# qwerty35/lsc_dr_planner

Hardware: AMD Instinct MI355X
Metric: qp_solves_per_sec (higher is better)
Workload: dtype f64; 1 GPU; configs[1]: 64 agents x M=5 x ~20 LSC half-spaces/seg, fp64 -- 64 agents/GPU x M=5 segments x 20 LSC neighbours (dim=3, forest swarm after 3 warm-up replans), fp64: dual active-set phase (one workgroup per QP) with the batched PDIP behind it for what it leaves; batch_seed=1000, precision=f64, row_format=f64, collective_backend=none (single process), agents_per_gpu=64, agents_total=64, ranks=1, distinct_devices=1, launch=single process, segments=5, lsc_neighbours=20, dim=3, rows_per_qp=1074, allgather=False, pipeline=False, hip_graph=False

## Files before the change

### lsc_dr_planner_amd/csrc/lscqp_das.hpp

```cpp
#pragma once
#include <hip/hip_runtime.h>
#include <stdint.h>

#include "lscqp_kernel.hpp"
#include "lscqp_launch.hpp"

#pragma clang fp contract(on)

namespace lscqp_das {

using lscqp::DevClass;
using lscqp::KQ;

constexpr double kTolP = 1e-9;
constexpr double kTolD = 1e-9;
constexpr int kMaxK = 32;

__host__ __device__ constexpr size_t table_stride(int M) { return (size_t)(3 + 6 * M) * (size_t)(6 * M); }
__host__ __device__ constexpr int num_pairs(int M, int dim) { return dim * (6 * M + 5 * M + 4 * M + M * (M - 1) / 2); }

struct Layout {
    int P, NX, kmax, NPAIR;
    int o_hdr, o_sfc, o_c, o_cu, o_lam, o_plo, o_phi, o_pix, o_W, o_L, o_u, o_r, o_arhs, o_acoef, o_aint, o_red, o_ctl, o_wb, o_dq, o_C, o_rows, o_tl, n_stage, total;
    __host__ __device__ static constexpr Layout make(int M, int dim, int kmax, int cacheC, int stage_rows = 0) {
        Layout s{};
        s.P = 6 * M, s.NX = dim * s.P, s.kmax = kmax, s.NPAIR = num_pairs(M, dim);
        int o = 0;
        auto take = [&](int n) { const int at = o; o += (n + 1) & ~1; return at; };
        s.o_hdr = take(32);
        s.o_sfc = take(6 * M);
        s.o_c = take(3 * s.P), s.o_cu = take(s.NX), s.o_lam = take(s.NX);
        s.o_plo = take(s.NPAIR), s.o_phi = take(s.NPAIR), s.o_pix = take((s.NPAIR + 1) / 2);
        s.o_W = take((kmax + 1) * s.NX);
        s.o_L = take(kmax * (kmax + 1));
        s.o_u = take(kmax + 1), s.o_r = take(kmax + 4), s.o_arhs = take(kmax + 1);
        s.o_acoef = take(3 * (kmax + 1));
        s.o_aint = take(2 * (kmax + 1) + 2);
        s.o_red = take(2 * 24);
        s.o_ctl = take(8);
        s.o_wb = take(8);
        s.o_dq = take(36);
        s.o_C = take(cacheC ? s.P * s.P : 0);
        s.n_stage = stage_rows;
        s.o_rows = take(4 * stage_rows);
#ifdef LSCQP_DAS_TIMING
        s.o_tl = take(16);
#endif
        s.total = o;
        return s;
    }
};

__device__ __forceinline__ double wave_max(double v) { return lscqp::wave_max(v); }
__device__ __forceinline__ double wave_min(double v) { return -lscqp::wave_max(-v); }
__device__ __forceinline__ double wave_sum(double v) { return lscqp::wave_sum(v); }
template <int CTRL, int ROW_MASK>
__device__ __forceinline__ int dpp_min_i32(int v) {
    return min(v, __builtin_amdgcn_update_dpp(2147483647, v, CTRL, ROW_MASK, 0xf, false));
}
__device__ __forceinline__ int wave_min_i32(int v) {
    v = dpp_min_i32<0x111, 0xf>(v);
    v = dpp_min_i32<0x112, 0xf>(v);
    v = dpp_min_i32<0x114, 0xf>(v);
    v = dpp_min_i32<0x118, 0xf>(v);
    v = dpp_min_i32<0x142, 0xa>(v);
    v = dpp_min_i32<0x143, 0xc>(v);
    return __builtin_amdgcn_readlane(v, 63);
}
__device__ __forceinline__ void wave_argmin(double& v, int& id) {
    const double vm = wave_min(v);
    id = wave_min_i32((v == vm) ? id : 2147483647);
    v = vm;
}
__device__ __forceinline__ int fdiv(int a, float inv_b) { return (int)(((float)a + 0.5f) * inv_b); }

#ifndef LSCQP_DAS_FULL_SYNC
#define LSCQP_DAS_WAVE_SYNC()                                   \
    do {                                                        \
        __builtin_amdgcn_fence(__ATOMIC_RELEASE, "wavefront");  \
        __builtin_amdgcn_wave_barrier();                        \
        __builtin_amdgcn_fence(__ATOMIC_ACQUIRE, "wavefront");  \
    } while (0)
#define LSCQP_DAS_BARRIER()                                                           \
    do {                                                                              \
        if constexpr (NW > 1) asm volatile("s_waitcnt lgkmcnt(0)\n\ts_barrier" ::: "memory"); \
        else asm volatile("s_waitcnt lgkmcnt(0)" ::: "memory");                       \
    } while (0)
#else
#define LSCQP_DAS_WAVE_SYNC()                                           \
    do {                                                                \
        __builtin_amdgcn_fence(__ATOMIC_SEQ_CST, "workgroup");          \
        asm volatile("s_waitcnt vmcnt(0) lgkmcnt(0)" ::: "memory");     \
        __builtin_amdgcn_wave_barrier();                                \
        __builtin_amdgcn_fence(__ATOMIC_SEQ_CST, "workgroup");          \
    } while (0)
#define LSCQP_DAS_BARRIER()                                             \
    do {                                                                \
        __builtin_amdgcn_fence(__ATOMIC_SEQ_CST, "workgroup");          \
        asm volatile("s_waitcnt vmcnt(0) lgkmcnt(0)" ::: "memory");     \
        if constexpr (NW > 1) __syncthreads();                          \
        __builtin_amdgcn_fence(__ATOMIC_SEQ_CST, "workgroup");          \
    } while (0)
#endif

#ifdef LSCQP_DAS_TIMING
#ifndef LSCQP_DAS_CYCLES
#define LSCQP_DAS_CYCLES das_cycles
#endif
__device__ unsigned long long LSCQP_DAS_CYCLES[16];
#define DAS_T_DECL()                                                                                                                  \
    unsigned long long* const das_tl_ = reinterpret_cast<unsigned long long*>(smem + L.o_tl);                                         \
    if (threadIdx.x == 0)                                                                                                             \
        for (int i_ = 0; i_ < 16; i_++) das_tl_[i_] = 0;                                                                              \
    unsigned long long tprev_ = __builtin_readcyclecounter()
#define DAS_T(slot)                                                        \
    do {                                                                   \
        if ((LSCQP_DAS_TIMING >> (slot)) & 1) {                            \
            const unsigned long long now_ = __builtin_readcyclecounter();  \
            if (tid == 0) das_tl_[slot] += now_ - tprev_;                  \
            tprev_ = now_;                                                 \
        }                                                                  \
    } while (0)
#ifndef LSCQP_DAS_TIMING_MIN_STEPS
#define LSCQP_DAS_TIMING_MIN_STEPS 0
#endif
#define DAS_T_FLUSH()                                                                    \
    do {                                                                                 \
        if (tid == 0 && steps >= LSCQP_DAS_TIMING_MIN_STEPS)                             \
            for (int i_ = 0; i_ < 16; i_++) atomicAdd(&LSCQP_DAS_CYCLES[i_], das_tl_[i_]);   \
    } while (0)
#else
#define DAS_T_DECL() \
    do {             \
    } while (0)
#define DAS_T(slot) \
    do {            \
    } while (0)
#define DAS_T_FLUSH() \
    do {              \
    } while (0)
#endif

#define LSCQP_DAS_GLOBAL __attribute__((address_space(1)))
#define LSCQP_DAS_KERNARGS()                                                                                                            \
    double ka_wb0 = cls.world_min[0], ka_wb1 = cls.world_min[1], ka_wb2 = cls.world_min[2];                                            \
    double ka_wb3 = cls.world_max[0], ka_wb4 = cls.world_max[1], ka_wb5 = cls.world_max[2];                                            \
    double ka_dt = cls.dt, ka_q2s = cls.q2s, ka_w_t = cls.w_t, ka_w_c = cls.w_c, ka_comm_range = cls.comm_range;                               \
    int ka_use_sfc = cls.use_sfc, ka_rsfc = cls.rsfc;                                                                                  \
    const int32_t* const ka_order = cls.order;                                                                                        \
    LSCQP_DAS_GLOBAL const uint64_t* ka_roffs = (LSCQP_DAS_GLOBAL const uint64_t*)row_offsets;                                         \
    LSCQP_DAS_GLOBAL const double* ka_sfc = (LSCQP_DAS_GLOBAL const double*)sfc;                                                       \
    asm volatile(""                                                                                                                    \
                 : "+s"(ka_wb0), "+s"(ka_wb1), "+s"(ka_wb2), "+s"(ka_wb3), "+s"(ka_wb4), "+s"(ka_wb5), "+s"(ka_dt), "+s"(ka_q2s),      \
                   "+s"(ka_w_t), "+s"(ka_w_c), "+s"(ka_comm_range), "+s"(ka_use_sfc), "+s"(ka_rsfc), "+s"(ka_roffs), "+s"(ka_sfc)                   \
                 : "s"(ka_order), "s"(tab), "s"(hdr), "s"(rows), "s"(n), "s"(cap), "s"(kmax), "s"(max_steps),        \
                   "s"(cacheC), "s"(stage_rows), "s"(x_init), "s"(x_out), "s"(obj_out), "s"(status_out), "s"(info_out))

struct Row {
    int ent[3];
    double coef[3];
    double rhs;
};
__device__ __forceinline__ int ent_axis(int e) { return e >> 16; }
__device__ __forceinline__ int ent_cp(int e) { return e & 0xffff; }

__device__ __forceinline__ double ccol(const int* ea, const double* ca, int kx, int cp, const double* __restrict__ Cm, int P) {
    double s = 0.0;
#pragma unroll
    for (int i = 0; i < 3; i++) {
        const double v = Cm[(size_t)ent_cp(ea[i]) * P + cp];
        s += ((ent_axis(ea[i]) == kx) ? ca[i] : 0.0) * v;
    }
    return s;
}
__device__ __forceinline__ double cdot(const int* ea, const double* ca, const int* eb, const double* cb, const double* __restrict__ Cm, int P) {
    double s = 0.0;
#pragma unroll
    for (int i = 0; i < 3; i++) {
#pragma unroll
        for (int j = 0; j < 3; j++) {
            const double v = Cm[(size_t)ent_cp(ea[i]) * P + ent_cp(eb[j])];
            s += ((ent_axis(ea[i]) == ent_axis(eb[j])) ? ca[i] * cb[j] : 0.0) * v;
        }
    }
    return s;
}

#ifndef LSCQP_DAS_KU1
#define LSCQP_DAS_KU1 2
#endif
#ifndef LSCQP_DAS_WPE1
#define LSCQP_DAS_WPE1 3
#endif
#ifndef LSCQP_DAS_WPES
#define LSCQP_DAS_WPES 4
#endif
enum DasVerdict { kDasSolved = 0, kDasInfeasible = 1, kDasHandedOver = 2 };

template <int NW, bool F32, bool SCREEN = false, bool PEEL = false>
__global__ __launch_bounds__(64 * NW, (SCREEN ? LSCQP_DAS_WPES : NW == 1 ? LSCQP_DAS_WPE1 : 1)) void das_kernel(DevClass cls, int M, int dim, int es, int cap, int kmax, int max_steps, int cacheC, int stage_rows, int behind,
                                                      const double* __restrict__ tab, int64_t n, const lscqp_header* __restrict__ hdr,
                                                      const lscqp_row* __restrict__ rows, const uint64_t* __restrict__ row_offsets,
                                                      const lscqp_box* __restrict__ sfc, const double* __restrict__ x_init, double* __restrict__ x_out,
                                                      double* __restrict__ obj_out, int32_t* __restrict__ status_out, lscqp_info* __restrict__ info_out) {
    extern __shared__ __attribute__((aligned(16))) double smem[];
    constexpr int T = 64 * NW;
    constexpr int kU = SCREEN ? 4 : (NW == 1) ? LSCQP_DAS_KU1 : 4;
    constexpr int kMaxNL = 0x7fffffff;
    const int64_t k0 = blockIdx.x;
    if (k0 >= n) return;
    const int64_t q = cls.order ? (int64_t)cls.order[k0] : k0;
#define LSCQP_DAS_PROLOGUE 0
#define LSCQP_DAS_STEP_PATH 0
#define LSCQP_DAS_END(verdict_) return
#include "lscqp_das_body.inc"
#undef LSCQP_DAS_END
#undef LSCQP_DAS_STEP_PATH
#undef LSCQP_DAS_PROLOGUE
}

}
```

### lsc_dr_planner_amd/csrc/lscqp_das_body.inc

```
#if LSCQP_DAS_PROLOGUE
#define DAS_CLS(f) ka_##f
#else
#define DAS_CLS(f) cls.f
#endif
    const int tid = threadIdx.x, lane = tid & 63, wv = tid >> 6;
#ifdef LSCQP_DAS_LAYOUT
    constexpr Layout L = LSCQP_DAS_LAYOUT;
#else
    const Layout L = Layout::make(M, dim, kmax, cacheC, stage_rows);
#endif
    DAS_T_DECL();
    const int P = L.P, NX = L.NX, NPAIR = L.NPAIR;
    const int kcap = L.kmax;
    double* const H_ = smem + L.o_hdr;
    double* const sfc_ = smem + L.o_sfc;
    double* const c_ = smem + L.o_c;
    double* const cu_ = smem + L.o_cu;
    double* const lam_ = smem + L.o_lam;
    double* const plo_ = smem + L.o_plo;
    double* const phi_ = smem + L.o_phi;
    int* const pix_ = reinterpret_cast<int*>(smem + L.o_pix);
    double* const W_ = smem + L.o_W;
    double* const Jm_ = smem + L.o_L;
    double* const u_ = smem + L.o_u;
// ... 138 lines not shown
    }
    const double dt = DAS_CLS(dt);
    const double org0 = Hd->p0[0], org1 = Hd->p0[1], org2 = Hd->p0[2];
    const double* const org = Hd->p0;
    int ts = Hd->terminal_segments;
    if (ts <= 0) {
        const double g0 = Hd->goal[0] - org0, g1 = Hd->goal[1] - org1, g2 = Hd->goal[2] - org2;
        ts = (int)((M * dt - sqrt(g0 * g0 + g1 * g1 + g2 * g2) / Hd->nominal_velocity + 1e-9) / dt);
        if (ts < 1) ts = 1;
    }
    if (ts > M) ts = M;
    const double q2s = DAS_CLS(q2s), wt2 = 2.0 * DAS_CLS(w_t);
    const double* const tb = tab + (size_t)(ts - 1) * table_stride(M);
    const double* const U1 = tb, * const U2 = tb + P, * const G1 = tb + 2 * P, * const Cg = tb + 3 * P;
    const bool comm_on = DAS_CLS(comm_range) > 0;
    const double rho_pair = 0.5 * DAS_CLS(comm_range) - Hd->radius;
    const double rho_wp = 0.5 * DAS_CLS(comm_range) - 1e-5;
#if !LSCQP_DAS_PROLOGUE
    const int nL = n_obs * P;
#endif
    const float iP = 1.0f / (float)P;
    const bool staged = stage_rows > 0 && nL <= stage_rows;
    bool rows_in_lds = false;

#if LSCQP_DAS_PROLOGUE
    constexpr int NE = 4;
    double tu1[NE], tu2[NE], tg1[NE];
#pragma unroll
    for (int i = 0; i < NE; i++) {
        const int e = tid + i * T < NX ? tid + i * T : 0;
        const int cp = e - P * fdiv(e, iP);
        tu1[i] = U1[cp], tu2[i] = U2[cp], tg1[i] = G1[cp];
    }
#else
    auto fetch_row = [&](int j, double& x, double& y, double& z, double& w) {
        if constexpr (F32) {
            const float4 f = reinterpret_cast<const float4*>(rows)[roff + (uint64_t)j];
            x = f.x, y = f.y, z = f.z, w = f.w;
        } else {
            const double4 d = *reinterpret_cast<const double4*>(&rows[roff + (uint64_t)j]);
            x = d.x, y = d.y, z = d.z, w = d.w;
        }
    };
    constexpr int NE = 4;
    double tu1[NE], tu2[NE], tg1[NE];
#pragma unroll
    for (int i = 0; i < NE; i++) {
        const int e = tid + i * T;
        if (e < NX) {
            const int cp = e - P * fdiv(e, iP);
            tu1[i] = U1[cp], tu2[i] = U2[cp], tg1[i] = G1[cp];
        }
    }
    double px[kU], py[kU], pz[kU], pw[kU];
#pragma unroll
    for (int u = 0; u < kU; u++) px[u] = py[u] = pz[u] = 0.0, pw[u] = -1.0;
    if (nL > 0) {
#pragma unroll
        for (int u = 0; u < kU; u++) {
            const int j = tid + u * T;
            fetch_row(j < nL ? j : 0, px[u], py[u], pz[u], pw[u]);
        }
    }
#endif

    constexpr int kCPre = (NW == 4 && !PEEL && !SCREEN) ? 6 : 0;
    double cpre[kCPre > 0 ? kCPre : 1];
#if LSCQP_DAS_PROLOGUE
    const bool c_fits = kCPre > 0 && P * P <= kCPre * T;
    const bool c_prefetched = c_fits && cacheC;
#else
    const bool c_prefetched = kCPre > 0 && cacheC && P * P <= kCPre * T;
    const bool c_fits = c_prefetched;
#endif
    if constexpr (kCPre > 0) {
        if (c_fits) {
#pragma unroll
            for (int i = 0; i < kCPre; i++) {
                const int e = tid + i * T;
                cpre[i] = Cg[e < P * P ? e : 0];
            }
        }
    }
#if LSCQP_DAS_STEP_PATH & 2
#ifndef LSCQP_DAS_LAYOUT
#error "LSCQP_DAS_STEP_PATH & 2 needs the compile-time carve"
#endif
    static_assert(NW > 1, "the first pass's barrier publishes the table");
    constexpr bool kTableEarly = kCPre > 0 && L.P * L.P <= kCPre * T;
    static_assert(!kTableEarly || LSCQP_DAS_PROLOGUE, "the table is stored from cpre[]: it needs the prologue that always loads it");
#else
    constexpr bool kTableEarly = false;
#endif

    bool empty = false;
    const double hv_c = dt * 0.2, ha_c = dt * dt * 0.05;
    for (int r0 = tid; r0 < NPAIR; r0 += kPB * T) {
        if (r0 != tid) {
#pragma unroll
            for (int u = 0; u < kPB; u++) pwr[u] = pairs_g[min(r0 + u * T, NPAIR - 1)];
        }
#pragma unroll
        for (int u = 0; u < kPB; u++) {
            if ((r0 - tid) + u * T >= NPAIR) break;
            const int r = r0 + u * T;
            const int w0 = pwr[u].x, w1 = pwr[u].y;
            const int fam = w1 & 3, k = (w1 >> 2) & 3, m = (w1 >> 4) & 15;
            const bool last = (w1 >> 8) & 1, rs = (w1 >> 9) & 1;
            const double ok_ = org[k], wlo = wb_[k], whi = wb_[3 + k], wpk = Hd->next_waypoint[k] - ok_;
            const double hv = Hd->vmax[k] * hv_c, ha = Hd->amax[k] * ha_c;
            double lo = wlo - ok_, hi = whi - ok_;
            if (DAS_CLS(rsfc) && rs) {
                lo = -100.0 - ok_;
                hi = 100.0 - ok_;
            }
            if (DAS_CLS(use_sfc)) {
                lo = fmax(lo, sfcl[m].bmin[k] - ok_);
                hi = fmin(hi, sfcl[m].bmax[k] - ok_);
            }
            const double clo = fmax(lo, fmax(-rho_pair, wpk - rho_wp)), chi = fmin(hi, fmin(rho_pair, wpk + rho_wp));
            lo = (comm_on && last) ? clo : lo;
            hi = (comm_on && last) ? chi : hi;
            const double hs = fam == 1 ? hv : fam == 2 ? ha : rho_pair;
            lo = fam == 0 ? lo : -hs;
            hi = fam == 0 ? hi : hs;
            if (r < NPAIR) {
                if (fam == 0 && (w0 >> 24) != 0 && lo > hi) empty = true;
                plo_[r] = lo, phi_[r] = hi;
                pix_[r] = w0;
            }
        }
    }
#pragma unroll
    for (int i = 0; i < NE; i++) {
        const int e = tid + i * T;
        if (e < NX) {
            const int k = fdiv(e, iP), cp = e - k * P;
            const double c1 = Hd->v0[k] * dt * 0.2;
            const double c2 = Hd->a0[k] * dt * dt * 0.05 + 2.0 * c1;
            const double fixv = (cp == 1) ? c1 : (cp == 2) ? c2 : 0.0;
            const double cv = fixv - c1 * tu1[i] - c2 * tu2[i] + wt2 * (Hd->goal[k] - org[k]) * tg1[i];
            c_[e] = cv;
            cu_[e] = cv;
        }
    }
    if (dim == 2)
        for (int e = tid; e < P; e += T) c_[2 * P + e] = 0.0;
#if LSCQP_DAS_STEP_PATH & 2
    {
        double2* const J2 = reinterpret_cast<double2*>(Jm_);
        for (int e = tid; e < kcap * LDL / 2; e += T) J2[e] = make_double2(0.0, 0.0);
    }
#endif
#if LSCQP_DAS_PROLOGUE
    const bool empty_w = __ballot(empty) != 0;
    if constexpr (NW > 1) {
        if (lane == 0) red_[20 + wv] = empty_w ? 1.0 : 0.0;
    }
    LSCQP_DAS_BARRIER();
    bool empty_g = empty_w;
    if constexpr (NW > 1) {
        empty_g = false;
#pragma unroll
        for (int w = 0; w < NW; w++) empty_g = empty_g || red_[20 + w] != 0.0;
    }
#else
    if (tid == 0) ctl_[4] = 0.0;
    LSCQP_DAS_BARRIER();
    if (empty) ctl_[4] = 1.0;
    LSCQP_DAS_BARRIER();
#endif
#if LSCQP_DAS_PROLOGUE
    if (empty_g)
#else
    if (ctl_[4] != 0.0)
#endif
    {
        double ov = 0.0;
        if (wv == 0) {
            for (int r = lane; r < NPAIR; r += 64)
                if ((pix_[r] >> 24) != 0) ov = fmax(ov, plo_[r] - phi_[r]);
            ov = wave_max(ov);
        }
        infeasible_out(0, ov);
        LSCQP_DAS_END(kDasInfeasible);
    }
    DAS_T(1);

    auto translate = [&](int j, double x, double y, double z, double w, double& nx, double& ny, double& nz, double& b) -> bool {
        nx = x, ny = y, nz = (dim == 3) ? z : 0.0;
        b = (dim == 3) ? w - (x * org0 + y * org1 + z * org2) : w - (x * org0 + y * org1 + 0.0);
        return !(x * x + y * y + z * z < 1e-10) && (j - P * fdiv(j, iP)) >= 3;
    };
    auto load_row = [&](int j, double& nx, double& ny, double& nz, double& b) -> bool {
        if (rows_in_lds) {
            nx = Sx_[j], ny = Sy_[j], nz = Sz_[j], b = Sb_[j];
            return b != -1.0 || nx != 0.0 || ny != 0.0 || nz != 0.0;
        }
        double x, y, z, w;
        fetch_row(j, x, y, z, w);
        return translate(j, x, y, z, w, nx, ny, nz, b);
    };
    auto pair_val = [&](int pk, const double* vec) -> double {
        const int type = pk >> 24, e0 = (pk >> 12) & 0xfff, e1 = pk & 0xfff;
        const int i0 = (type == 4) ? e1 : e0 + max(type - 1, 0);
        const int i1 = (type == 3) ? e0 + 1 : e0;
        const double a1 = (type <= 1) ? 0.0 : (type == 3) ? -2.0 : -1.0;
        const double a2 = (type == 3) ? 1.0 : 0.0;
        const double v0 = vec[i0], v1 = vec[i1], v2 = vec[e0];
        return (v0 + a1 * v1) + a2 * v2;
    };
    auto ent_of = [&](int e) -> int {
        const int k = fdiv(e, iP);
        return (k << 16) | (e - k * P);
    };
    auto decode = [&](int rid, Row& R) {
        R.ent[0] = R.ent[1] = R.ent[2] = 0;
        R.coef[0] = R.coef[1] = R.coef[2] = 0.0;
        if (rid < nL) {
            const int cp = rid - P * fdiv(rid, iP);
            double nx, ny, nz, b;
            (void)load_row(rid, nx, ny, nz, b);
            R.ent[0] = cp, R.ent[1] = (1 << 16) | cp, R.ent[2] = (2 << 16) | cp;
            R.coef[0] = nx, R.coef[1] = ny, R.coef[2] = (dim == 3) ? nz : 0.0;
            R.rhs = b;
            return;
        }
        const int s = rid - nL, r = s >> 1, pk = pix_[r];
        const int type = pk >> 24, e0 = (pk >> 12) & 0xfff, e1 = pk & 0xfff;
        const double sg = (s & 1) ? -1.0 : 1.0;
        R.rhs = (s & 1) ? -phi_[r] : plo_[r];
        const bool t1 = type == 1, t2 = type == 2, t3 = type == 3;
        R.ent[0] = ent_of(t1 ? e0 : t2 ? e0 + 1 : t3 ? e0 + 2 : e1);
        R.ent[1] = t1 ? 0 : ent_of(t3 ? e0 + 1 : e0);
        R.ent[2] = t3 ? ent_of(e0) : 0;
        R.coef[0] = sg;
        R.coef[1] = t1 ? 0.0 : t3 ? -2.0 * sg : -sg;
        R.coef[2] = t3 ? sg : 0.0;
    };
    auto row_dot = [&](const int* ent, const double* coef, const double* vec) -> double {
        return coef[0] * vec[ent_axis(ent[0]) * P + ent_cp(ent[0])] + coef[1] * vec[ent_axis(ent[1]) * P + ent_cp(ent[1])] +
               coef[2] * vec[ent_axis(ent[2]) * P + ent_cp(ent[2])];
    };

    bool first_pass = true;
    auto pass_local = [&](double& bv, int& bi) {
        bv = 1e300;
        bi = 0x7fffffff;
        auto see = [&](double slack, int id) {
            slack = (slack == slack) ? slack : -1e308;
            const bool lt = slack < bv;
            bv = lt ? slack : bv;
            bi = lt ? id : bi;
        };
        auto eval = [&](int j0, const double* rx, const double* ry, const double* rz, const double* rb) {
#pragma unroll
            for (int u = 0; u < kU; u++) {
                const int j = j0 + u * T, jc = j < nL ? j : 0;
                const int cp = jc - P * fdiv(jc, iP);
                see(rx[u] * c_[cp] + ry[u] * c_[P + cp] + rz[u] * c_[2 * P + cp] - rb[u], j);
            }
        };
        auto prep = [&](int j0, const double* x, const double* y, const double* z, const double* w, double* rx, double* ry, double* rz, double* rb) {
#pragma unroll
            for (int u = 0; u < kU; u++) {
                const int j = j0 + u * T, jc = j < nL ? j : 0;
                const bool ok = translate(jc, x[u], y[u], z[u], w[u], rx[u], ry[u], rz[u], rb[u]) && j < nL;
                rx[u] = ok ? rx[u] : 0.0, ry[u] = ok ? ry[u] : 0.0, rz[u] = ok ? rz[u] : 0.0, rb[u] = ok ? rb[u] : -1.0;
            }
        };
        auto stage = [&](int j0, const double* rx, const double* ry, const double* rz, const double* rb) {
#pragma unroll
            for (int u = 0; u < kU; u++) {
                const int j = j0 + u * T;
                if (j < nL) Sx_[j] = rx[u], Sy_[j] = ry[u], Sz_[j] = rz[u], Sb_[j] = rb[u];
            }
        };
        double rx[kU], ry[kU], rz[kU], rb[kU];
        if (first_pass) {
            prep(tid, px, py, pz, pw, rx, ry, rz, rb);
            if (staged) stage(tid, rx, ry, rz, rb);
            eval(tid, rx, ry, rz, rb);
            for (int j0 = tid + kU * T; kMaxNL > kU * T && j0 < nL; j0 += kU * T) {
                double x[kU], y[kU], z[kU], w[kU];
#pragma unroll
                for (int u = 0; u < kU; u++) fetch_row(j0 + u * T < nL ? j0 + u * T : 0, x[u], y[u], z[u], w[u]);
                prep(j0, x, y, z, w, rx, ry, rz, rb);
                if (staged) stage(j0, rx, ry, rz, rb);
                eval(j0, rx, ry, rz, rb);
            }
        } else if (rows_in_lds) {
#if LSCQP_DAS_STEP_PATH & 1
            for (int j0 = tid; j0 < nL; j0 += kU * T) {
                double lx[kU], ly[kU], lz[kU], lb[kU];
#pragma unroll
                for (int u = 0; u < kU; u++) {
                    const int j = j0 + u * T, jc = j < nL ? j : 0;
                    lx[u] = Sx_[jc], ly[u] = Sy_[jc], lz[u] = Sz_[jc], lb[u] = Sb_[jc];
                }
#pragma unroll
                for (int u = 0; u < kU; u++) {
                    const bool in = j0 + u * T < nL;
                    rx[u] = in ? lx[u] : 0.0, ry[u] = in ? ly[u] : 0.0, rz[u] = in ? lz[u] : 0.0, rb[u] = in ? lb[u] : -1.0;
                }
                eval(j0, rx, ry, rz, rb);
            }
#else
            for (int j0 = tid; j0 < nL; j0 += kU * T) {
#pragma unroll
                for (int u = 0; u < kU; u++) {
                    const int j = j0 + u * T, jc = j < nL ? j : 0;
                    rx[u] = Sx_[jc], ry[u] = Sy_[jc], rz[u] = Sz_[jc], rb[u] = (j < nL) ? Sb_[jc] : 1e300;
                    if (!(j < nL)) rx[u] = ry[u] = rz[u] = 0.0, rb[u] = -1.0;
                }
                eval(j0, rx, ry, rz, rb);
            }
#endif
        } else {
            for (int j0 = tid; j0 < nL; j0 += kU * T) {
                double x[kU], y[kU], z[kU], w[kU];
#pragma unroll
                for (int u = 0; u < kU; u++) fetch_row(j0 + u * T < nL ? j0 + u * T : 0, x[u], y[u], z[u], w[u]);
                prep(j0, x, y, z, w, rx, ry, rz, rb);
                eval(j0, rx, ry, rz, rb);
            }
        }
        first_pass = false;
        DAS_T(8);
        for (int r0 = tid; r0 < NPAIR; r0 += 2 * T) {
            const int r1 = r0 + T, r1c = r1 < NPAIR ? r1 : r0;
            const int pk0 = pix_[r0], pk1 = pix_[r1c];
            const double lo0 = plo_[r0], hi0 = phi_[r0], lo1 = plo_[r1c], hi1 = phi_[r1c];
            const double d0 = pair_val(pk0, c_), d1 = pair_val(pk1, c_);
            const bool on0 = (pk0 >> 24) != 0, on1 = (pk1 >> 24) != 0 && r1 < NPAIR;
            see(on0 ? d0 - lo0 : 1.0, nL + 2 * r0);
            see(on0 ? hi0 - d0 : 1.0, nL + 2 * r0 + 1);
            see(on1 ? d1 - lo1 : 1.0, nL + 2 * r1);
            see(on1 ? hi1 - d1 : 1.0, nL + 2 * r1 + 1);
        }
        DAS_T(9);
    };
    auto pass_combine = [&](const double* rb_, double& bv, int& bi) {
        bv = rb_[0], bi = reinterpret_cast<const int*>(rb_ + 4)[0];
#pragma unroll
        for (int w = 1; w < NW; w++) {
            const double ov = rb_[w];
            const int oi = reinterpret_cast<const int*>(rb_ + 4)[w];
            if (ov < bv || (ov == bv && oi < bi)) bv = ov, bi = oi;
        }
    };
    auto pass = [&](double& best, int& bid) {
        const bool was_first = first_pass;
        double bv;
        int bi;
        pass_local(bv, bi);
#if LSCQP_DAS_STEP_PATH & 2
        if constexpr (kTableEarly) {
            if (was_first) {
#pragma unroll
                for (int i = 0; i < kCPre; i++) {
                    const int e = tid + i * T;
                    if (e < P * P) Cc_[e] = cpre[i];
                }
            }
        }
#endif
        wave_argmin(bv, bi);
        if constexpr (NW > 1) {
            double* const rb_ = red_ + 24 * par;
            par ^= 1;
            if (lane == 0) {
                rb_[wv] = bv;
                reinterpret_cast<int*>(rb_ + 4)[wv] = bi;
            }
            LSCQP_DAS_BARRIER();
            pass_combine(rb_, bv, bi);
        } else if (staged && was_first) {
            LSCQP_DAS_BARRIER();
        }
        if (staged) rows_in_lds = true;
        best = bv, bid = bi;
    };

    const double* Cm = kTableEarly ? Cc_ : Cg;
    auto factor_remove = [&](int k_, int l_) -> bool {
        bool ok = true;
        if (wv == 0) {
            const int k = __builtin_amdgcn_readfirstlane(k_), l = __builtin_amdgcn_readfirstlane(l_);
            const bool mine = lane < k;
            const int c = mine ? lane : 0;
            const int cn = c - (c > l ? 1 : 0);
            double carry = Jm_[l * LDL + c];
            double a = Jm_[l * LDL + l];
            for (int j = l; j < k - 1; j++) {
                const double x = Jm_[(j + 1) * LDL + c];
                const double b = Jm_[(j + 1) * LDL + l];
                const double r2 = a * a + b * b;
                if (!(r2 > 1e-280)) ok = false;
                const double ir = rsqrt(fmax(r2, 1e-300));
                const double ca = a * ir, sb = b * ir;
                const double fin = ca * x - sb * carry;
                carry = ca * carry + sb * x;
                a = r2 * ir;
                if (mine && lane != l) Jm_[j * LDL + cn] = fin;
            }
            if (mine) Jm_[(k - 1) * LDL + lane] = 0.0, Jm_[lane * LDL + k - 1] = 0.0;
            LSCQP_DAS_WAVE_SYNC();
        }
        return ok;
    };
    auto solve_factor = [&](int k_, double vi, double* yy) -> double {
        const int k = __builtin_amdgcn_readfirstlane(k_);
        const bool mine = lane < k;
        const int ll = min(lane, kcap - 1);
        vi = mine ? vi : 0.0;
        double yi = 0.0, ri = 0.0;
        for (int j0 = 0; j0 < k; j0 += 8) {
            double Jr[8];
#pragma unroll
            for (int t_ = 0; t_ < 8; t_++) Jr[t_] = Jm_[ll * LDL + min(j0 + t_, kcap)];
#pragma unroll
            for (int t_ = 0; t_ < 8; t_++) yi += Jr[t_] * lscqp::bcast(vi, j0 + t_);
        }
        yi = mine ? yi : 0.0;
        if (yy) *yy = wave_sum(yi * yi);
        for (int j0 = 0; j0 < k; j0 += 8) {
            double Jc[8];
#pragma unroll
            for (int t_ = 0; t_ < 8; t_++) Jc[t_] = Jm_[min(j0 + t_, kcap - 1) * LDL + ll];
#pragma unroll
            for (int t_ = 0; t_ < 8; t_++) ri += Jc[t_] * lscqp::bcast(yi, j0 + t_);
        }
        ri = mine ? ri : 0.0;
        if (lane < kcap + 4) r_[lane] = ri;
        return ri;
    };
    auto add_columns = [&](int k, const double* wts, const double* base) {
        for (int e = tid; e < NX; e += T) {
            double a = base ? base[e] : c_[e];
            for (int j = 0; j < k; j++) a += wts[j] * W_[(size_t)j * NX + e];
            c_[e] = a;
        }
    };

    const int NZA = 3 * (M - 1) + (es ? 1 : 3);
    auto finish_local = [&](int k, double& rd, double& gs, double& part) {
#if LSCQP_DAS_PROLOGUE
        const double dt = wb_[6], q2s = wb_[7], ka_w_t = ctl_[4], ka_w_c = red_[44], wt2 = 2.0 * ka_w_t;
#endif
        if (k > 0) {
            for (int e = tid; e < NX; e += T) lam_[e] = 0.0;
            LSCQP_DAS_BARRIER();
            if (tid == 0) {
                for (int j = 0; j < k; j++)
#pragma unroll
                    for (int t_ = 0; t_ < 3; t_++) {
                        const int en = aint_[4 * j + 1 + t_];
                        lam_[ent_axis(en) * P + ent_cp(en)] += u_[j] * acoef_[3 * j + t_];
                    }
            }
            LSCQP_DAS_BARRIER();
        }
        rd = 0.0, gs = 0.0;
        for (int zi = tid; zi < dim * NZA; zi += T) {
            const int kx = zi / NZA, a = zi - kx * NZA;
            const bool last = es && a == 3 * (M - 1);
            const int m = last ? M - 1 : a / 3, j = last ? 0 : a % 3;
            const double c1 = Hd->v0[kx] * dt * 0.2;
            const double c2 = Hd->a0[kx] * dt * dt * 0.05 + 2.0 * c1;
            const double gk = Hd->goal[kx] - org[kx];
            auto seg = [&](int mm, double* g, double* g0, double* lm) {
                const double* cc = &c_[kx * P + 6 * mm];
                const double v0 = cc[0], v1 = cc[1], v2 = cc[2], v3 = cc[3], v4 = cc[4], v5 = cc[5];
                lscqp::static_for<0, 6>([&](auto Ic) {
                    constexpr int i = decltype(Ic)::value;
                    g[i] = q2s * (KQ(i, 0) * v0 + KQ(i, 1) * v1 + KQ(i, 2) * v2 + KQ(i, 3) * v3 + KQ(i, 4) * v4 + KQ(i, 5) * v5);
                    g0[i] = (mm == 0) ? q2s * (KQ(i, 1) * c1 + KQ(i, 2) * c2) : 0.0;
                    lm[i] = (k > 0) ? lam_[kx * P + 6 * mm + i] : 0.0;
                });
                if (mm >= M - ts) {
                    g[5] += wt2 * (v5 - gk);
                    g0[5] += -wt2 * gk;
                }
            };
            double g[6], g0[6], lm[6];
            seg(m, g, g0, lm);
            double cf, cg, c0;
            if (last) {
                cf = (g[3] - lm[3]) + (g[4] - lm[4]) + (g[5] - lm[5]), cg = g[3] + g[4] + g[5], c0 = g0[3] + g0[4] + g0[5];
            } else {
                const double gs_ = j == 0 ? g[3] : j == 1 ? g[4] : g[5], ls_ = j == 0 ? lm[3] : j == 1 ? lm[4] : lm[5], g0s = j == 0 ? g0[3] : j == 1 ? g0[4] : g0[5];
                cf = gs_ - ls_, cg = gs_, c0 = g0s;
            }
            if (m + 1 < M) {
                seg(m + 1, g, g0, lm);
                const double w0 = (j == 2) ? 1.0 : 0.0, w1 = (j == 1) ? -1.0 : (j == 2) ? 2.0 : 0.0, w2 = (j == 0) ? 1.0 : (j == 1) ? -4.0 : 4.0;
                cf += w0 * (g[0] - lm[0]) + w1 * (g[1] - lm[1]) + w2 * (g[2] - lm[2]);
                cg += w0 * g[0] + w1 * g[1] + w2 * g[2];
                c0 += w0 * g0[0] + w1 * g0[1] + w2 * g0[2];
            }
            rd = fmax(rd, fabs(cf));
            gs = fmax(gs, fmax(fabs(cg), fabs(c0)));
        }
        part = 0.0;
        for (int lv = tid - (NW > 1 ? 64 : 0); lv < dim * M; lv += T) {
            if (lv < 0) continue;
            const int kx = lv / M, m = lv - kx * M;
            const double* cc = &c_[kx * P + 6 * m];
            const double j0 = (cc[3] - cc[0]) - 3.0 * (cc[2] - cc[1]);
            const double j1 = (cc[4] - cc[1]) - 3.0 * (cc[3] - cc[2]);
            const double j2 = (cc[5] - cc[2]) - 3.0 * (cc[4] - cc[3]);
            const double quad = 0.2 * (j0 * j0 + j2 * j2) + (2.0 / 15.0) * j1 * j1 + 0.2 * (j0 * j1 + j1 * j2) + (1.0 / 15.0) * j0 * j2;
            double pp = 0.5 * q2s * 3600.0 * quad;
            const double ok_ = org[kx];
            double corr = 0;
            const double s0 = cc[0] + ok_, s1 = cc[1] + ok_, s2 = cc[2] + ok_, s3 = cc[3] + ok_, s4 = cc[4] + ok_, s5 = cc[5] + ok_;
#pragma unroll 1
            for (int i = 0; i < 6; i++) {
                const double* dr = dq_ + 6 * i;
                double r = 0;
                r += dr[0] * s0, r += dr[1] * s1, r += dr[2] * s2, r += dr[3] * s3, r += dr[4] * s4, r += dr[5] * s5;
                corr += r * (cc[i] + ok_);
            }
            pp += DAS_CLS(w_c) * corr;
            const double dgoal = cc[5] - (Hd->goal[kx] - ok_);
            pp += (m >= M - ts) ? DAS_CLS(w_t) * dgoal * dgoal : 0.0;
            part += pp;
        }
    };
    auto finish_combine = [&](const double* rb_, double& rd, double& gs, double& part) {
        rd = rb_[8], gs = rb_[12], part = rb_[16];
#pragma unroll
        for (int w = 1; w < NW; w++) rd = fmax(rd, rb_[8 + w]), gs = fmax(gs, rb_[12 + w]), part += rb_[16 + w];
    };
    auto finish_verdict = [&](double rd, double gs, double part, double& res_d, double& obj) {
        res_d = (part == part && fabs(part) < 1e300) ? rd / fmax(1.0, gs) : 1e300;
        obj = part;
    };
    auto finish = [&](int k, double& res_d, double& obj) {
        double rd, gs, part;
        finish_local(k, rd, gs, part);
        lscqp::wave_reduce3<lscqp::OpMax, lscqp::OpMax, lscqp::OpSum>(rd, gs, part);
        if constexpr (NW > 1) {
            double* const rb_ = red_ + 24 * par;
            par ^= 1;
            if (lane == 0) rb_[8 + wv] = rd, rb_[12 + wv] = gs, rb_[16 + wv] = part;
            LSCQP_DAS_BARRIER();
            finish_combine(rb_, rd, gs, part);
        }
        finish_verdict(rd, gs, part, res_d, obj);
    };

    int k = 0, steps = 0, why = LSCQP_DAS_WHY_VERIFICATION;
    bool polished = false, solved = false, haveC = false, haveJ = false, proven = false;
    double res_p = 0.0, res_d = 0.0, obj = 0.0;
    auto write_out = [&]() {
        for (int e = tid; e < NX; e += T) x_out[q * NX + e] = c_[e] + org[fdiv(e, iP)];
        if (tid == 0) {
            obj_out[q] = obj;
            status_out[q] = LSCQP_STATUS_OPTIMAL;
            if (info_out) {
                info_out[q].iterations = steps;
                info_out[q].flags = LSCQP_INFO_ACTIVE_SET;
                info_out[q].res_primal = res_p;
                info_out[q].res_dual = res_d;
                info_out[q].gap = 0.0;
            }
        }
    };
    double best;
    int bid;
    bool peeled = false;
    if constexpr (PEEL || SCREEN) {
        pass(best, bid);
        DAS_T(2);
        if (!(best < -kTolP)) {
            res_p = fmax(0.0, -best);
            finish(0, res_d, obj);
            DAS_T(4);
            if (res_d <= kTolD) write_out();
            else hand_over(0, LSCQP_DAS_WHY_VERIFICATION);
            DAS_T(7);
            DAS_T_FLUSH();
            LSCQP_DAS_END(res_d <= kTolD ? kDasSolved : kDasHandedOver);
        }
        peeled = true;
    }
    for (;;) {
        if (!((PEEL || SCREEN) && peeled)) {
            pass(best, bid);
            DAS_T(steps == 0 ? 2 : 3);
        }
        peeled = false;
        if (!(best < -kTolP)) {
            res_p = fmax(0.0, -best);
            finish(k, res_d, obj);
            DAS_T(4);
            if (res_d <= kTolD) {
                solved = true;
                break;
            }
            if (polished || k == 0) break;
            LSCQP_DAS_BARRIER();
            add_columns(k, u_, cu_);
            LSCQP_DAS_BARRIER();
            if (wv == 0) {
                const double rho = (lane < k) ? arhs_[lane] - row_dot(&aint_[4 * lane + 1], &acoef_[3 * lane], c_) : 0.0;
                const double du = solve_factor(k, rho, nullptr);
                const double un = (lane < k) ? u_[lane] + du : 0.0;
                const double umax = wave_max(fabs(un));
                const double neg = wave_max((lane < k && un < -1e-12 * umax) ? 1.0 : 0.0);
                if (lane < k) u_[lane] = fmax(un, 0.0);
                if (lane == 0) ctl_[7] = neg;
            }
            LSCQP_DAS_BARRIER();
            if (ctl_[7] != 0.0) {
                why = LSCQP_DAS_WHY_MULTIPLIER;
                break;
            }
            add_columns(k, r_, nullptr);
            LSCQP_DAS_BARRIER();
            polished = true;
            continue;
        }
        polished = false;
        if constexpr (SCREEN) break;
        if (k >= kmax) {
            why = LSCQP_DAS_WHY_ROWS;
            break;
        }
#if LSCQP_DAS_STEP_PATH & 2
        (void)haveJ, (void)haveC;
#else
        if (!haveJ) {
            if (wv == 0)
                for (int e = lane; e < kcap * LDL; e += 64) Jm_[e] = 0.0;
            haveJ = true;
        }
#endif
        if (!kTableEarly && cacheC && !haveC) {
            bool copied = false;
            if constexpr (kCPre > 0) {
                if (c_prefetched) {
#pragma unroll
                    for (int i = 0; i < kCPre; i++) {
                        const int e = tid + i * T;
                        if (e < P * P) Cc_[e] = cpre[i];
                    }
                    copied = true;
                }
            }
            if (!copied)
                for (int e = tid; e < P * P; e += T) Cc_[e] = Cg[e];
            haveC = true;
            Cm = Cc_;
            LSCQP_DAS_BARRIER();
        }
        Row Rp;
        decode(bid, Rp);
        if (tid == 0) {
            aint_[4 * kcap] = bid;
            for (int t = 0; t < 3; t++) aint_[4 * kcap + 1 + t] = Rp.ent[t], acoef_[3 * kcap + t] = Rp.coef[t];
            arhs_[kcap] = Rp.rhs;
            ctl_[3] = 0.0;
        }
        auto compute_wp = [&](int first_thread, int n_threads) {
            for (int e = tid - first_thread; e < NX; e += n_threads) {
                if (e < 0) continue;
                const int kx = fdiv(e, iP), cp = e - kx * P;
                W_[(size_t)k * NX + e] = ccol(Rp.ent, Rp.coef, kx, cp, Cm, P);
            }
        };
        if constexpr (NW == 1) compute_wp(0, T);
        DAS_T(5);
        double spp = 0.0;
        bool stop = false, first_step = true;
        for (;;) {
            steps++;
            if (steps > max_steps) {
                stop = true;
                why = LSCQP_DAS_WHY_STEPS;
                break;
            }
            if (NW > 1 && first_step && wv != 0) compute_wp(64, T - 64);
            if (wv == 0 && __builtin_amdgcn_readfirstlane(k) == 0) {
                if (first_step) spp = cdot(Rp.ent, Rp.coef, Rp.ent, Rp.coef, Cm, P);
                const double sp = row_dot(Rp.ent, Rp.coef, c_) - Rp.rhs;
                const double t = (spp > 1e-12 * spp) ? -sp / spp : 1e300;
                const int kind = (t < 1e299) ? 1 : 0;
                if (lane == 0) {
                    if (kind == 1) Jm_[0] = rsqrt(spp), u_[0] = ctl_[3] + t;
                    ctl_[0] = t;
                    ctl_[1] = (double)kind;
                    ctl_[2] = 0.0;
                    ctl_[3] += t;
                    ctl_[5] = (t < 1e299) ? 1.0 : 0.0;
                }
            } else if (wv == 0) {
                if (first_step) spp = cdot(Rp.ent, Rp.coef, Rp.ent, Rp.coef, Cm, P);
                const double vj = (lane < k) ? row_dot(Rp.ent, Rp.coef, W_ + (size_t)lane * NX) : 0.0;
                DAS_T(13);
                double yy;
                const double ri = solve_factor(k, vj, &yy);
                DAS_T(14);
                const double curv = spp - yy;
                const double sp = row_dot(Rp.ent, Rp.coef, c_) - Rp.rhs;
                const double t2 = (curv > 1e-12 * spp) ? -sp / curv : 1e300;
                double t1 = (lane < k && ri > 0.0) ? u_[lane] / ri : 1e300;
                int l = lane;
                wave_argmin(t1, l);
                const double t = fmin(t1, t2);
                int kind;
                if (!(t < 1e299)) kind = (sp < -1e-6) ? 3 : 0;
                else if (t2 <= t1) kind = 1;
                else kind = 2;
                DAS_T(15);
                if (kind == 1 || kind == 2) {
                    if (lane < k) u_[lane] = fmax(0.0, u_[lane] - t * ri);
                    if (kind == 1) {
                        const double idl = rsqrt(curv);
                        if (lane < k) Jm_[k * LDL + lane] = -ri * idl, Jm_[lane * LDL + k] = 0.0;
                        if (lane == 0) Jm_[k * LDL + k] = idl, u_[k] = ctl_[3] + t;
                    }
                }
                if (lane == 0) {
                    ctl_[0] = t;
                    ctl_[1] = (double)kind;
                    ctl_[2] = (double)l;
                    ctl_[3] += t;
                    ctl_[5] = (t2 < 1e299) ? 1.0 : 0.0;
                    ctl_[7] = -sp;
                }
            }
            first_step = false;
            DAS_T(10);
            LSCQP_DAS_BARRIER();
            const double t = ctl_[0];
            const int kind = __builtin_amdgcn_readfirstlane((int)ctl_[1]), l = __builtin_amdgcn_readfirstlane((int)ctl_[2]);
            if (kind == 0 || kind == 3) {
                stop = true;
                why = LSCQP_DAS_WHY_NO_STEP;
                proven = kind == 3;
                break;
            }
            const int ks = __builtin_amdgcn_readfirstlane(k);
            const bool primal = __builtin_amdgcn_readfirstlane((int)ctl_[5]) != 0;
            for (int e = tid; e < NX; e += T) {
                if (primal) {
                    double a = W_[(size_t)ks * NX + e];
                    for (int j0 = 0; j0 < ks; j0 += 4) {
                        double wj[4], rj[4];
#pragma unroll
                        for (int t_ = 0; t_ < 4; t_++)
                            wj[t_] = W_[(size_t)min(j0 + t_, ks) * NX + e], rj[t_] = r_[j0 + t_];
#pragma unroll
// ... 89 lines not shown
```

### lsc_dr_planner_amd/csrc/lscqp_fused.hip

```cpp
#include <atomic>

#include "lscqp_kernel.hpp"
#include "lscqp_launch.hpp"
#define LSCQP_DAS_CYCLES das_fused_cycles
#include "lscqp_das.hpp"

#define LSCQP_FCAT_(a, b, c, d, e, f) a##b##_##c##_##d##_##e##_##f
#define LSCQP_FCAT(a, b, c, d, e, f) LSCQP_FCAT_(a, b, c, d, e, f)
#define LSCQP_FUSED_FN LSCQP_FCAT(lscqp_launch_fused_, LSCQP_M, LSCQP_DIM, LSCQP_ES, LSCQP_NSLOT, LSCQP_W)

namespace lscqp_das {

constexpr bool carve_fits(int M, int dim, int kmax, int stage_rows) {
    return sizeof(double) * (size_t)Layout::make(M, dim, kmax, 1, stage_rows).total <= lscqp::kMaxLdsBytes;
}
#if LSCQP_M == 10 && LSCQP_DIM == 3
#define LSCQP_FUSED_PROLOGUE 0
#else
#define LSCQP_FUSED_PROLOGUE 1
#endif
#ifndef LSCQP_FUSED_STEP_PATH
#if LSCQP_M == 5
#define LSCQP_FUSED_STEP_PATH 7
#else
#define LSCQP_FUSED_STEP_PATH 0
#endif
#endif
template <int M, int DIM, bool ES, int NSLOT, int W>
struct FusedCarve {
    static constexpr int kStage = lscqp::Cfg<M, DIM, ES, NSLOT, W, (int)sizeof(double)>::MAX_OBS * 6 * M;
    static constexpr int KMAX = carve_fits(M, DIM, kMaxK, kStage) ? kMaxK : 20;
    static_assert(carve_fits(M, DIM, KMAX, kStage), "the fused phase's carve does not fit the CU's LDS");
};

template <int M, int DIM, bool ES, int NSLOT, int W>
__global__ __launch_bounds__(256, 1) void das_pdip_kernel(DevClass cls, int cap, int kmax, int max_steps, int cacheC, int stage_rows,
                                                          const double* __restrict__ tab, int64_t n, const lscqp_header* __restrict__ hdr,
                                                          const lscqp_row* __restrict__ rows, const uint64_t* __restrict__ row_offsets,
                                                          const lscqp_box* __restrict__ sfc, const double* __restrict__ x_init,
                                                          double* __restrict__ x_out, double* __restrict__ obj_out, int32_t* __restrict__ status_out,
                                                          lscqp_info* __restrict__ info_out) {
    static_assert(W >= 1 && W <= 4, "the interior-point instance runs on the first W of the workgroup's four wavefronts");
    extern __shared__ __attribute__((aligned(16))) double smem[];
#if LSCQP_FUSED_PROLOGUE
    LSCQP_DAS_KERNARGS();
    const int64_t k0 = blockIdx.x;
    if (k0 >= n) return;
    const int64_t q = ka_order ? (int64_t)ka_order[k0] : k0;
#else
    const int64_t k0 = blockIdx.x;
    if (k0 >= n) return;
    const int64_t q = cls.order ? (int64_t)cls.order[k0] : k0;
#endif
    int verdict = kDasSolved;
    {
        constexpr int NW = 4, T = 64 * NW, kU = 4;
        constexpr bool F32 = false, SCREEN = false, PEEL = false;
        constexpr int dim = DIM, es = ES ? 1 : 0, behind = 0;
        using FC = FusedCarve<M, DIM, ES, NSLOT, W>;
        constexpr int kMaxNL = FC::kStage;
#define LSCQP_DAS_END(verdict_)   \
    do {                          \
        verdict = (verdict_);     \
        goto phase_done;          \
    } while (0)
#define LSCQP_DAS_LAYOUT Layout::make(M, DIM, FC::KMAX, 1, FC::kStage)
#define LSCQP_DAS_PROLOGUE LSCQP_FUSED_PROLOGUE
#define LSCQP_DAS_STEP_PATH LSCQP_FUSED_STEP_PATH
#include "lscqp_das_body.inc"
#undef LSCQP_DAS_STEP_PATH
#undef LSCQP_DAS_PROLOGUE
#undef LSCQP_DAS_LAYOUT
#undef LSCQP_DAS_END
    }
phase_done:
    verdict = __builtin_amdgcn_readfirstlane(verdict);
    if (verdict != kDasHandedOver) return;
    __syncthreads();
    if constexpr (W < 4) {
        if (__builtin_amdgcn_readfirstlane((int)(threadIdx.x >> 6)) >= W) return;
    }
    lscqp::lscqp_pdip_one<M, DIM, ES, NSLOT, W, double>(cls, q, smem, hdr, rows, row_offsets, sfc, x_init, x_out, obj_out, status_out, info_out);
}

}

extern "C" hipError_t LSCQP_FUSED_FN(const lscqp::DevClass* cls, int cap, int kmax, int max_steps, int cacheC, int stage_rows, const double* d_tab,
                                     int64_t n, const lscqp_header* hdr, const lscqp_row* rows, const uint64_t* row_offsets, const lscqp_box* sfc,
                                     const double* x_init, double* x_out, double* obj_out, int32_t* status_out, lscqp_info* info_out,
                                     hipStream_t stream) {
    using C = lscqp::Cfg<LSCQP_M, LSCQP_DIM, (LSCQP_ES != 0), LSCQP_NSLOT, LSCQP_W, (int)sizeof(double)>;
    using FC = lscqp_das::FusedCarve<LSCQP_M, LSCQP_DIM, (LSCQP_ES != 0), LSCQP_NSLOT, LSCQP_W>;
    auto kern = lscqp_das::das_pdip_kernel<LSCQP_M, LSCQP_DIM, (LSCQP_ES != 0), LSCQP_NSLOT, LSCQP_W>;
    if (kmax < 1 || kmax > lscqp_das::kMaxK || cls->rows_f32 || cls->queue || cls->scan || cls->repair != 3) return hipErrorInvalidValue;
    if (cls->n_obs_max > C::MAX_OBS || cap > C::MAX_OBS) return hipErrorNotSupported;
    if (kmax > FC::KMAX || stage_rows > FC::kStage) return hipErrorNotSupported;
    const size_t lds_das = sizeof(double) * (size_t)lscqp_das::Layout::make(LSCQP_M, LSCQP_DIM, FC::KMAX, 1, FC::kStage).total;
    const size_t lds = lds_das > C::lds_bytes() ? lds_das : C::lds_bytes();
    if (lds > lscqp::kMaxLdsBytes) return hipErrorNotSupported;
    static std::atomic<bool> attr_set[64];
    int dev = 0;
    if (hipGetDevice(&dev) != hipSuccess || dev < 0 || dev >= 64) return hipErrorInvalidDevice;
    if (!attr_set[dev].load(std::memory_order_acquire)) {
        const hipError_t e = hipFuncSetAttribute(reinterpret_cast<const void*>(kern), hipFuncAttributeMaxDynamicSharedMemorySize, (int)lscqp::kMaxLdsBytes);
        if (e != hipSuccess) return e;
        attr_set[dev].store(true, std::memory_order_release);
    }
    if (n <= 0) return hipSuccess;
    hipLaunchKernelGGL(kern, dim3((unsigned)n), dim3(256), lds, stream, *cls, cap, kmax, max_steps, cacheC, stage_rows, d_tab, n, hdr, rows, row_offsets, sfc,
                       x_init, x_out, obj_out, status_out, info_out);
    return hipGetLastError();
}

#ifdef LSCQP_DAS_TIMING
extern "C" int lscqp_das_fused_cycles(unsigned long long* out, int reset) {
    (void)hipMemcpyFromSymbol(out, HIP_SYMBOL(lscqp_das::das_fused_cycles), sizeof(unsigned long long) * 16);
    if (reset) {
        unsigned long long z[16] = {0};
        (void)hipMemcpyToSymbol(HIP_SYMBOL(lscqp_das::das_fused_cycles), z, sizeof z);
    }
    return 0;
}
#endif
```

Measured before the change: 6.818 million QP/s.

## Restructure DAS stationarity check to drop lam clearing barrier and parallelize objective

Adds a step-path bit that clears the multiplier vector once in the prologue and then only zeroes the touched entries after each active-set step, which removes a full clear-plus-barrier from each finish pass. The stationarity residual is computed per constraint row in registers by the first wavefronts, and the objective moves onto the second wavefront with its coefficients held in registers. The row-slot count kU now follows from the staged row count. The new path is enabled for M=5 and for M=10 with dim 2. The timing macro gains a configurable thread id. The change adds code complexity and relies on lam_ staying zeroed between steps.

```diff
diff --git a/lsc_dr_planner_amd/csrc/lscqp_das.hpp b/lsc_dr_planner_amd/csrc/lscqp_das.hpp
--- a/lsc_dr_planner_amd/csrc/lscqp_das.hpp
+++ b/lsc_dr_planner_amd/csrc/lscqp_das.hpp
@@ -108,16 +108,19 @@
 #define LSCQP_DAS_CYCLES das_cycles
 #endif
 __device__ unsigned long long LSCQP_DAS_CYCLES[16];
+#ifndef LSCQP_DAS_TIMING_TID
+#define LSCQP_DAS_TIMING_TID 0
+#endif
 #define DAS_T_DECL()                                                                                                                  \
     unsigned long long* const das_tl_ = reinterpret_cast<unsigned long long*>(smem + L.o_tl);                                         \
-    if (threadIdx.x == 0)                                                                                                             \
+    if (threadIdx.x == LSCQP_DAS_TIMING_TID)                                                                                          \
         for (int i_ = 0; i_ < 16; i_++) das_tl_[i_] = 0;                                                                              \
     unsigned long long tprev_ = __builtin_readcyclecounter()
 #define DAS_T(slot)                                                        \
     do {                                                                   \
         if ((LSCQP_DAS_TIMING >> (slot)) & 1) {                            \
             const unsigned long long now_ = __builtin_readcyclecounter();  \
-            if (tid == 0) das_tl_[slot] += now_ - tprev_;                  \
+            if (tid == LSCQP_DAS_TIMING_TID) das_tl_[slot] += now_ - tprev_; \
             tprev_ = now_;                                                 \
         }                                                                  \
     } while (0)
@@ -126,7 +129,7 @@
 #endif
 #define DAS_T_FLUSH()                                                                    \
     do {                                                                                 \
-        if (tid == 0 && steps >= LSCQP_DAS_TIMING_MIN_STEPS)                             \
+        if (tid == LSCQP_DAS_TIMING_TID && steps >= LSCQP_DAS_TIMING_MIN_STEPS)          \
             for (int i_ = 0; i_ < 16; i_++) atomicAdd(&LSCQP_DAS_CYCLES[i_], das_tl_[i_]);   \
     } while (0)
 #else
diff --git a/lsc_dr_planner_amd/csrc/lscqp_das_body.inc b/lsc_dr_planner_amd/csrc/lscqp_das_body.inc
--- a/lsc_dr_planner_amd/csrc/lscqp_das_body.inc
+++ b/lsc_dr_planner_amd/csrc/lscqp_das_body.inc
@@ -314,6 +314,9 @@
         for (int e = tid; e < kcap * LDL / 2; e += T) J2[e] = make_double2(0.0, 0.0);
     }
 #endif
+#if LSCQP_DAS_STEP_PATH & 8
+    for (int e = tid; e < NX; e += T) lam_[e] = 0.0;
+#endif
 #if LSCQP_DAS_PROLOGUE
     const bool empty_w = __ballot(empty) != 0;
     if constexpr (NW > 1) {
@@ -610,6 +613,157 @@
 #if LSCQP_DAS_PROLOGUE
         const double dt = wb_[6], q2s = wb_[7], ka_w_t = ctl_[4], ka_w_c = red_[44], wt2 = 2.0 * ka_w_t;
 #endif
+#if LSCQP_DAS_STEP_PATH & 8
+#if !LSCQP_DAS_PROLOGUE
+#error "LSCQP_DAS_STEP_PATH & 8 reads the class's scalars from LDS: it needs the rescheduled prologue"
+#endif
+        static_assert(NW > 1, "the stationarity rows take one trip of the workgroup");
+        auto objective_local = [&]() {
+#if LSCQP_DAS_STEP_PATH & 32
+            static_assert(NW > 1, "the objective's lanes are the second wavefront's");
+            part = 0.0;
+            if (__builtin_amdgcn_readfirstlane(wv) == 1) {
+                const bool on = lane < dim * M;
+                const int lv = on ? lane : dim * M - 1;
+                const int kx = lv / M, m = lv - kx * M;
+                const double* cc = &c_[kx * P + 6 * m];
+                double cv[6], dqv[36];
+                double ok_ = org[kx], gl_ = Hd->goal[kx];
+#pragma unroll
+                for (int i = 0; i < 6; i++) cv[i] = cc[i];
+#pragma unroll
+                for (int i = 0; i < 36; i++) dqv[i] = dq_[i];
+                asm volatile("" : "+v"(ok_), "+v"(gl_));
+#pragma unroll
+                for (int i = 0; i < 6; i++) asm volatile("" : "+v"(cv[i]));
+#pragma unroll
+                for (int i = 0; i < 36; i++) asm volatile("" : "+v"(dqv[i]));
+                const double j0 = (cv[3] - cv[0]) - 3.0 * (cv[2] - cv[1]);
+                const double j1 = (cv[4] - cv[1]) - 3.0 * (cv[3] - cv[2]);
+                const double j2 = (cv[5] - cv[2]) - 3.0 * (cv[4] - cv[3]);
+                const double quad = 0.2 * (j0 * j0 + j2 * j2) + (2.0 / 15.0) * j1 * j1 + 0.2 * (j0 * j1 + j1 * j2) + (1.0 / 15.0) * j0 * j2;
+                double pp = 0.5 * q2s * 3600.0 * quad;
+                double corr = 0;
+                const double s0 = cv[0] + ok_, s1 = cv[1] + ok_, s2 = cv[2] + ok_, s3 = cv[3] + ok_, s4 = cv[4] + ok_, s5 = cv[5] + ok_;
+#pragma unroll
+                for (int i = 0; i < 6; i++) {
+                    const double* dr = dqv + 6 * i;
+                    double r = 0;
+                    r += dr[0] * s0, r += dr[1] * s1, r += dr[2] * s2, r += dr[3] * s3, r += dr[4] * s4, r += dr[5] * s5;
+                    corr += r * (cv[i] + ok_);
+                }
+                pp += DAS_CLS(w_c) * corr;
+                const double dgoal = cv[5] - (gl_ - ok_);
+                pp += (m >= M - ts) ? DAS_CLS(w_t) * dgoal * dgoal : 0.0;
+                const double sum = part + pp;
+                part = on ? sum : part;
+            }
+#else
+            part = 0.0;
+            for (int lv = tid - (NW > 1 ? 64 : 0); lv < dim * M; lv += T) {
+                if (lv < 0) continue;
+                const int kx = lv / M, m = lv - kx * M;
+                const double* cc = &c_[kx * P + 6 * m];
+                const double j0 = (cc[3] - cc[0]) - 3.0 * (cc[2] - cc[1]);
+                const double j1 = (cc[4] - cc[1]) - 3.0 * (cc[3] - cc[2]);
+                const double j2 = (cc[5] - cc[2]) - 3.0 * (cc[4] - cc[3]);
+                const double quad = 0.2 * (j0 * j0 + j2 * j2) + (2.0 / 15.0) * j1 * j1 + 0.2 * (j0 * j1 + j1 * j2) + (1.0 / 15.0) * j0 * j2;
+                double pp = 0.5 * q2s * 3600.0 * quad;
+                const double ok_ = org[kx];
+                double corr = 0;
+                const double s0 = cc[0] + ok_, s1 = cc[1] + ok_, s2 = cc[2] + ok_, s3 = cc[3] + ok_, s4 = cc[4] + ok_, s5 = cc[5] + ok_;
+#pragma unroll 1
+                for (int i = 0; i < 6; i++) {
+                    const double* dr = dq_ + 6 * i;
+                    double r = 0;
+                    r += dr[0] * s0, r += dr[1] * s1, r += dr[2] * s2, r += dr[3] * s3, r += dr[4] * s4, r += dr[5] * s5;
+                    corr += r * (cc[i] + ok_);
+                }
+                pp += DAS_CLS(w_c) * corr;
+                const double dgoal = cc[5] - (Hd->goal[kx] - ok_);
+                pp += (m >= M - ts) ? DAS_CLS(w_t) * dgoal * dgoal : 0.0;
+                part += pp;
+            }
+#endif
+        };
+        const int nz = dim * NZA;
+        const bool zw = __builtin_amdgcn_readfirstlane(wv) * 64 < nz;
+        const bool zon = tid < nz;
+        const int zi = zon ? tid : nz - 1;
+        const int kx = zi / NZA, a = zi - kx * NZA;
+        const bool last = es && a == 3 * (M - 1);
+        const int m = last ? M - 1 : a / 3, j = last ? 0 : a % 3;
+        const bool has_next = m + 1 < M;
+        const int mn = has_next ? m + 1 : M - 1;
+        double hv0, ha0, hgl, hok, va[6], vb[6];
+        if (zw) {
+            hv0 = Hd->v0[kx], ha0 = Hd->a0[kx], hgl = Hd->goal[kx], hok = org[kx];
+#pragma unroll
+            for (int i = 0; i < 6; i++) va[i] = c_[kx * P + 6 * m + i], vb[i] = c_[kx * P + 6 * mn + i];
+        }
+        if (k > 0) {
+            if (tid == 0) {
+                for (int j_ = 0; j_ < k; j_++)
+#pragma unroll
+                    for (int t_ = 0; t_ < 3; t_++) {
+                        const int en = aint_[4 * j_ + 1 + t_];
+                        lam_[ent_axis(en) * P + ent_cp(en)] += u_[j_] * acoef_[3 * j_ + t_];
+                    }
+            }
+            LSCQP_DAS_BARRIER();
+        }
+        objective_local();
+        rd = 0.0, gs = 0.0;
+        if (zw) {
+            double la[3], lb[3];
+#pragma unroll
+            for (int i = 0; i < 3; i++) la[i] = lam_[kx * P + 6 * m + 3 + i], lb[i] = lam_[kx * P + 6 * mn + i];
+            double dt_ = dt, q2s_ = q2s, wt2_ = wt2;
+            asm volatile("" : "+v"(hv0), "+v"(ha0), "+v"(hgl), "+v"(hok), "+v"(dt_), "+v"(q2s_), "+v"(wt2_));
+#pragma unroll
+            for (int i = 0; i < 6; i++) asm volatile("" : "+v"(va[i]), "+v"(vb[i]));
+#pragma unroll
+            for (int i = 0; i < 3; i++) asm volatile("" : "+v"(la[i]), "+v"(lb[i]));
+            {
+                const double dt = dt_, q2s = q2s_, wt2 = wt2_;
+                const double c1 = hv0 * dt * 0.2;
+                const double c2 = ha0 * dt * dt * 0.05 + 2.0 * c1;
+                const double gk = hgl - hok;
+                auto seg = [&](int mm, const double* cc, double* g, double* g0) {
+                    const double v0 = cc[0], v1 = cc[1], v2 = cc[2], v3 = cc[3], v4 = cc[4], v5 = cc[5];
+                    lscqp::static_for<0, 6>([&](auto Ic) {
+                        constexpr int i = decltype(Ic)::value;
+                        g[i] = q2s * (KQ(i, 0) * v0 + KQ(i, 1) * v1 + KQ(i, 2) * v2 + KQ(i, 3) * v3 + KQ(i, 4) * v4 + KQ(i, 5) * v5);
+                        g0[i] = (mm == 0) ? q2s * (KQ(i, 1) * c1 + KQ(i, 2) * c2) : 0.0;
+                    });
+                    if (mm >= M - ts) {
+                        g[5] += wt2 * (v5 - gk);
+                        g0[5] += -wt2 * gk;
+                    }
+                };
+                double g[6], g0[6];
+                seg(m, va, g, g0);
+                const double lm3 = la[0], lm4 = la[1], lm5 = la[2];
+                double cf, cg, c0;
+                {
+                    const double cf_l = (g[3] - lm3) + (g[4] - lm4) + (g[5] - lm5), cg_l = g[3] + g[4] + g[5], c0_l = g0[3] + g0[4] + g0[5];
+                    const double gs_ = j == 0 ? g[3] : j == 1 ? g[4] : g[5], ls_ = j == 0 ? lm3 : j == 1 ? lm4 : lm5, g0s = j == 0 ? g0[3] : j == 1 ? g0[4] : g0[5];
+                    cf = last ? cf_l : gs_ - ls_, cg = last ? cg_l : gs_, c0 = last ? c0_l : g0s;
+                }
+                {
+                    seg(mn, vb, g, g0);
+                    const double* const lm = lb;
+                    const double w0 = (j == 2) ? 1.0 : 0.0, w1 = (j == 1) ? -1.0 : (j == 2) ? 2.0 : 0.0, w2 = (j == 0) ? 1.0 : (j == 1) ? -4.0 : 4.0;
+                    const double cf_n = cf + (w0 * (g[0] - lm[0]) + w1 * (g[1] - lm[1]) + w2 * (g[2] - lm[2]));
+                    const double cg_n = cg + (w0 * g[0] + w1 * g[1] + w2 * g[2]);
+                    const double c0_n = c0 + (w0 * g0[0] + w1 * g0[1] + w2 * g0[2]);
+                    cf = has_next ? cf_n : cf, cg = has_next ? cg_n : cg, c0 = has_next ? c0_n : c0;
+                }
+                const double rd_ = fmax(rd, fabs(cf)), gs_z = fmax(gs, fmax(fabs(cg), fabs(c0)));
+                rd = zon ? rd_ : rd, gs = zon ? gs_z : gs;
+            }
+        }
+#else
         if (k > 0) {
             for (int e = tid; e < NX; e += T) lam_[e] = 0.0;
             LSCQP_DAS_BARRIER();
@@ -689,6 +843,7 @@
             pp += (m >= M - ts) ? DAS_CLS(w_t) * dgoal * dgoal : 0.0;
             part += pp;
         }
+#endif
     };
     auto finish_combine = [&](const double* rb_, double& rd, double& gs, double& part) {
         rd = rb_[8], gs = rb_[12], part = rb_[16];
@@ -763,6 +918,16 @@
                 break;
             }
             if (polished || k == 0) break;
+#if LSCQP_DAS_STEP_PATH & 8
+            if (tid == 0) {
+                for (int j_ = 0; j_ < k; j_++)
+#pragma unroll
+                    for (int t_ = 0; t_ < 3; t_++) {
+                        const int en = aint_[4 * j_ + 1 + t_], at = ent_axis(en) * P + ent_cp(en);
+                        if (at < NX) lam_[at] = 0.0;
+                    }
+            }
+#endif
             LSCQP_DAS_BARRIER();
             add_columns(k, u_, cu_);
             LSCQP_DAS_BARRIER();
diff --git a/lsc_dr_planner_amd/csrc/lscqp_fused.hip b/lsc_dr_planner_amd/csrc/lscqp_fused.hip
--- a/lsc_dr_planner_amd/csrc/lscqp_fused.hip
+++ b/lsc_dr_planner_amd/csrc/lscqp_fused.hip
@@ -20,8 +20,8 @@
 #define LSCQP_FUSED_PROLOGUE 1
 #endif
 #ifndef LSCQP_FUSED_STEP_PATH
-#if LSCQP_M == 5
-#define LSCQP_FUSED_STEP_PATH 7
+#if LSCQP_M == 5 || (LSCQP_M == 10 && LSCQP_DIM == 2)
+#define LSCQP_FUSED_STEP_PATH (7 | 8 | 32)
 #else
 #define LSCQP_FUSED_STEP_PATH 0
 #endif
@@ -54,11 +54,18 @@
 #endif
     int verdict = kDasSolved;
     {
-        constexpr int NW = 4, T = 64 * NW, kU = 4;
+        using FC = FusedCarve<M, DIM, ES, NSLOT, W>;
+        constexpr int NW = 4, T = 64 * NW;
+#ifdef LSCQP_FUSED_ROW_SLOTS
+        constexpr int kU = LSCQP_FUSED_ROW_SLOTS;
+#else
+        constexpr int kU = (FC::kStage + T - 1) / T < 4 ? (FC::kStage + T - 1) / T : 4;
+#endif
         constexpr bool F32 = false, SCREEN = false, PEEL = false;
         constexpr int dim = DIM, es = ES ? 1 : 0, behind = 0;
-        using FC = FusedCarve<M, DIM, ES, NSLOT, W>;
         constexpr int kMaxNL = FC::kStage;
+        static_assert(kU == 4 || kMaxNL <= kU * T, "the row slots must cover the carve's staged rows");
+        static_assert(kU >= 1, "an instance has rows");
 #define LSCQP_DAS_END(verdict_)   \
     do {                          \
         verdict = (verdict_);     \
```

After: 7.274 million QP/s (median of 6 runs). +6.7%, better.
